# danbider/gp-quadrature

Measured on AMD Instinct MI355X. Metric: GP-fits/sec (fit + posterior mean at the N training points), N=1e6 d=2 SE kernel, higher is better.
Workload: dtype f64; 1 GPU; 2D squared-exponential l=0.2 var=2 sigma2=0.2, eps=1e-4, global N=1e6 synthetic (BASELINE configs[1] at the metric's N=1e6), points sharded over the GPUs; n_per_gpu=1000000, global_n=1000000, d=2, mtot=23, M=529, mean_cg_iters=68, parallelism=points sharded over 1 GPU(s), CG replicated

## Files before the change

### gp-quadrature_amd/csrc/cg_herm.hip

```cpp
#include <cstdlib>
#include <type_traits>

#include "cg_persistent_dev.hpp"
#include "spectral_weights.hpp"

namespace efgp {

namespace pcg {

namespace h64 {
constexpr int kThreadsH = 256, kWavesH = kThreadsH / 64;
constexpr int LDR = 72;
constexpr int LT = 40;
constexpr int LQ = 82;
constexpr int G_ELEMS = 16 * LDR, T_ELEMS = 32 * LT, Q_ELEMS = kWavesH * 8 * LQ;
constexpr int kLdsElems = G_ELEMS + T_ELEMS + Q_ELEMS;

__device__ __forceinline__ void dft8_in4_tail(double2 e0, double2 e1, double2 e2, double2 e3, double2 o0, double2 o1r, double2 o2r,
                                              double2 o3r, double2 (&v)[8]) {
    const double hh = 0.70710678118654752440;
    const double2 o1 = make_double2(hh * (o1r.x + o1r.y), hh * (o1r.y - o1r.x));
    const double2 o2 = mul_mi(o2r);
    const double2 o3 = make_double2(hh * (o3r.y - o3r.x), -hh * (o3r.x + o3r.y));
    v[0] = cadd(e0, o0);
// ... 320 lines not shown
    double2* const qw = Qb + (wave * 8 + ql) * LQ + 9 * jc;
    const double2* const qr = Qb + (wave * 8 + ql) * LQ + jc;

    double2 twr[7], twc[7];
#pragma unroll
    for (int t = 1; t < 8; ++t) {
        twr[t - 1] = a.g.tw[0][j * t];
        twc[t - 1] = a.g.tw[0][jc * t];
    }
    double sa[8], sb[8];
#pragma unroll
    for (int t = 0; t < 8; ++t) {
        const int f0 = jc + 8 * t;
        const double2 va = a.vhat[f0 * F + q], vb = a.vhat[f0 * F + q + 32];
        const double2 wa = a.g.tw[0][((n - 1) * (f0 + q)) & 63], wb = a.g.tw[0][((n - 1) * (f0 + q + 32)) & 63];
        sa[t] = 0.5 * (va.x * wa.x + va.y * wa.y);
        sb[t] = -0.5 * (vb.x * wb.x + vb.y * wb.y);
    }
    const bool z6_ok = jc > 0;

    hrow::RowLanes<8> L;
    L.setup<false>(a, row_role, k0, j);
    const double (&wsr)[KS] = L.wsr;

#ifdef EFGP_CG_STAMPS
    long long stamp_prev = (long long)__builtin_readcyclecounter();
#endif
    int stop = 0;
    double rcp_rz = 0.0;
    auto apply_A = [&](const double2 (&u)[KS], double2 (&Au)[KS]) __attribute__((always_inline)) {
        double2 v[8];
        EFGP_STAMP(7);
        if (row_role) {
            dft8_in4(make_double2(wsr[0] * u[0].x, wsr[0] * u[0].y), make_double2(wsr[1] * u[1].x, wsr[1] * u[1].y),
                     make_double2(wsr[2] * u[2].x, wsr[2] * u[2].y), make_double2(wsr[3] * u[3].x, wsr[3] * u[3].y), v);
            exchange_stage2(v, xw, xr, twr);
            s64::store8_all<8>(Gb + k0 * LDR + j, v);
        }
        __syncthreads();
        stop = s_stop;
        rcp_rz = s_rcp;
        if (stop) return;
        EFGP_STAMP(0);
        {
            const double2* g0 = Gb + q;
            const double2 a0 = g0[jc * LDR], b0 = g0[jc * LDR + 32];
            const double2 a1 = g0[(jc + 8) * LDR], b1 = g0[(jc + 8) * LDR + 32];
            const double2 a6 = g0[((16 - jc) & 15) * LDR], b6 = g0[((16 - jc) & 15) * LDR + 32];
            const double2 a7 = g0[(8 - jc) * LDR], b7 = g0[(8 - jc) * LDR + 32];
            const double2 z0 = jc == 0 ? make_double2(a0.x, b0.x) : make_double2(a0.x - b0.y, a0.y + b0.x);
            const double2 z1 = make_double2(a1.x - b1.y, a1.y + b1.x);
            double2 z6 = make_double2(a6.x + b6.y, b6.x - a6.y);
            const double2 z7 = make_double2(a7.x + b7.y, b7.x - a7.y);
            if (!z6_ok) z6 = make_double2(0.0, 0.0);
            dft8_in4(z0, z1, z6, z7, v);
            exchange_stage2(v, qw, qr, twc);
#pragma unroll
            for (int t = 0; t < 8; ++t) v[t] = make_double2(v[t].x * sa[t], v[t].y * sb[t]);
            dft_fwd<8>(v);
            exchange_stage2<true>(v, qw, qr, twc);
            double2* t0 = Tb + jc * LT + q;
            t0[0] = v[0];
            t0[8 * LT] = v[1];
            t0[16 * LT] = v[6];
            t0[24 * LT] = v[7];
        }
        __syncthreads();
        EFGP_STAMP(1);
        if (row_role) {
            const double2* tp = Tb + (k0 & 15) * LT + j;
            const double2* tm = Tb + ((k0 & 15) == 0 ? 0 : 32 - (k0 & 15)) * LT + j;
#pragma unroll
            for (int u4 = 0; u4 < 4; ++u4) {
                const double2 P = tp[8 * u4], Mv = tm[8 * u4];
                v[u4] = make_double2(P.x + Mv.x, P.y - Mv.y);
                v[u4 + 4] = make_double2(-P.y - Mv.y, P.x - Mv.x);
            }
            dft_fwd<8>(v);
            exchange_stage2<true>(v, xw, xr, twr);
            const double2 y[KS] = {s64::conjd(v[0]), s64::conjd(v[1]), s64::conjd(v[6]), s64::conjd(v[7])};
#pragma unroll
            for (int s = 0; s < KS; ++s) {
                const double2 gg = make_double2(wsr[s] * y[s].x, wsr[s] * y[s].y);
                if (VARIANT == 0) Au[s] = make_double2(gg.x + a.sigmasq * u[s].x, gg.y + a.sigmasq * u[s].y);
                else Au[s] = make_double2(gg.x / a.sigmasq + u[s].x, gg.y / a.sigmasq + u[s].y);
            }
        } else {
#pragma unroll
            for (int s = 0; s < KS; ++s) Au[s] = make_double2(0.0, 0.0);
        }
        EFGP_STAMP(2);
    };

    if (tid == 0) {
        s_stop = 0;
        s_rcp = 0.0;
    }
    double2 Ap[KS];
    if (a.zero_x0) {
#pragma unroll
        for (int s = 0; s < KS; ++s) Ap[s] = make_double2(0.0, 0.0);
    } else {
        apply_A(L.xv, Ap);
    }
    double rz, bb, asym;
    L.start(a, Ap, rz, bb, asym);
    block_sum_pair_h(rz, bb, red);
    asym = block_sum_h(asym, red);
    const double ws_bad = block_sum_h(L.ws_bad, red + kWavesH);
    if (hrow::refused(asym, bb, ws_bad)) {
        L.refuse(a);
        return;
    }
    const hrow::NormTest norm(bb);
    if (wave == 3 && lane == 0) s_rcp = 1.0 / (rz + 1e-16);
    int it = 0;
    for (; it < a.max_iter;) {
        apply_A(L.pv, Ap);
        if (stop) break;
        const double pAp = block_sum_h(L.dot_p(Ap), red) + 1e-16;
        EFGP_STAMP(3);
        const double alpha = rz / pAp;
        double rr, rzn;
        double2 zv[KS];
        L.step(alpha, Ap, zv, rr, rzn);
        EFGP_STAMP(4);
        block_sum_pair_h(rr, rzn, red);
        EFGP_STAMP(5);
        ++it;
        if (wave == 3) norm.publish(a, rr, rzn, it, lane, &s_rcp, &s_stop);
        L.new_direction(zv, rzn, rz, rcp_rz);
    }
    L.write_out(a, it);
}

namespace h48 {
constexpr int kThreadsH = 256, kWavesH = kThreadsH / 64;
constexpr int HF = 24, NR = 12;
constexpr int LDR = 56;
constexpr int LT = 28;
constexpr int LQ = 82;
constexpr int G_ELEMS = NR * LDR, T_ELEMS = 2 * NR * LT, Q_ELEMS = HF * LQ;
static_assert(NR * LX <= Q_ELEMS, "the row lines' scratch aliases the column lines' scratch");
constexpr int kLdsElems = G_ELEMS + T_ELEMS + Q_ELEMS;
constexpr int ND = 4 * F;
constexpr int NC = 25;
constexpr int kReread = 8;
constexpr int LDV = 49;
constexpr int kLdsElemsDense = F * LDV + (kThreadsH / 8) * LX;
static_assert(2 * G_ELEMS + NR * LX <= kLdsElemsDense, "the iteration's G, Yh and row scratch alias the prologue's grid");
constexpr int kThreadsP = 512, kRowWavesP = 2, kPairWavesP = 3;
constexpr int NDP = kThreadsP - 64 * kRowWavesP;
static_assert(NDP == 8 * F && 64 * kPairWavesP == 4 * F, "no wave mixes two-row and one-row groups");
constexpr int kLdsElemsPairs = F * LDV + (kThreadsP / 8) * LX;

__device__ __forceinline__ void exchange_8to6(const double2 (&v)[8], double2 (&u)[6], bool writer, double2* __restrict__ wr,
                                              const double2* __restrict__ rd, const double2 (&tw)[5]) {
    wave_sync();
    if (writer) s64::store8_all<1>(wr, v);
    wave_sync();
#pragma unroll
    for (int t = 0; t < 6; ++t) u[t] = rd[9 * t];
#pragma unroll
    for (int t = 1; t < 6; ++t) u[t] = cmulp(u[t], tw[t - 1]);
    dft6(u);
}
__device__ __forceinline__ double exchange_8to6_norm(const double2 (&v)[8], double2 (&u)[6], bool writer, double2* __restrict__ wr,
                                                     const double2* __restrict__ rd, const double2 (&tw)[5], const double2 (&x)[4],
                                                     double scale) {
    wave_sync();
    if (writer) s64::store8_all<1>(wr, v);
    wave_sync();
#pragma unroll
    for (int t = 0; t < 6; ++t) u[t] = rd[9 * t];
    __builtin_amdgcn_sched_barrier(0);
    const double x01 = fma(x[0].x, x[0].x, x[0].y * x[0].y) + fma(x[1].x, x[1].x, x[1].y * x[1].y);
    const double x23 = fma(x[2].x, x[2].x, x[2].y * x[2].y) + fma(x[3].x, x[3].x, x[3].y * x[3].y);
    const double xx = scale * (x01 + x23);
    __builtin_amdgcn_sched_barrier(0);
#pragma unroll
    for (int t = 1; t < 6; ++t) u[t] = cmulp(u[t], tw[t - 1]);
    dft6(u);
    return xx;
}
__device__ __forceinline__ void exchange_6to8(double2 (&u)[6], double2 (&v)[8], double2* __restrict__ wr, const double2* __restrict__ rd,
                                              const double2 (&tw)[5]) {
#pragma unroll
    for (int t = 1; t < 6; ++t) u[t] = cmulp(u[t], tw[t - 1]);
    wave_sync();
#pragma unroll
    for (int t = 0; t < 6; ++t) wr[t] = u[t];
    wave_sync();
    s64::load8_all<9>(rd, v);
    h64::dft8_out4(v);
}

__device__ __forceinline__ double half_wave_sum(double v) {
    EFGP_DPP_ADD(v, 0x111, 0xF);
    EFGP_DPP_ADD(v, 0x112, 0xF);
    EFGP_DPP_ADD(v, 0x114, 0xF);
    EFGP_DPP_ADD(v, 0x118, 0xF);
    EFGP_DPP_ADD(v, 0x142, 0xA);
    const int lo = __builtin_amdgcn_readlane(__double2loint(v), 31);
    const int hi = __builtin_amdgcn_readlane(__double2hiint(v), 31);
    return __hiloint2double(hi, lo);
}

template <bool LOW_ROUNDED>
__device__ __forceinline__ void dft8_in4_ws(const double (&w)[4], const double2 (&u)[4], double2 (&v)[8]) {
    constexpr int r0 = LOW_ROUNDED ? 0 : 2, r1 = LOW_ROUNDED ? 1 : 3, f0 = LOW_ROUNDED ? 2 : 0, f1 = LOW_ROUNDED ? 3 : 1;
    double2 e0, e1, e2, e3, o0, o1r, o2r, o3r;
    const double2 ra = make_double2(__dmul_rn(w[r0], u[r0].x), __dmul_rn(w[r0], u[r0].y));
    const double2 rb = make_double2(__dmul_rn(w[r1], u[r1].x), __dmul_rn(w[r1], u[r1].y));
    const double wa = w[f0], wb = w[f1];
    const double2 ua = u[f0], ub = u[f1];
    if constexpr (LOW_ROUNDED) {
        e0 = make_double2(fma(wa, ua.x, ra.x), fma(wa, ua.y, ra.y));
        e1 = make_double2(fma(-wa, ua.y, ra.x), fma(wa, ua.x, ra.y));
        e2 = make_double2(fma(-wa, ua.x, ra.x), fma(-wa, ua.y, ra.y));
        e3 = make_double2(fma(wa, ua.y, ra.x), fma(-wa, ua.x, ra.y));
        o0 = make_double2(fma(wb, ub.x, rb.x), fma(wb, ub.y, rb.y));
        o1r = make_double2(fma(-wb, ub.y, rb.x), fma(wb, ub.x, rb.y));
        o2r = make_double2(fma(-wb, ub.x, rb.x), fma(-wb, ub.y, rb.y));
        o3r = make_double2(fma(wb, ub.y, rb.x), fma(-wb, ub.x, rb.y));
    } else {
        e0 = make_double2(fma(wa, ua.x, ra.x), fma(wa, ua.y, ra.y));
        e1 = make_double2(fma(wa, ua.x, -ra.y), fma(wa, ua.y, ra.x));
        e2 = make_double2(fma(wa, ua.x, -ra.x), fma(wa, ua.y, -ra.y));
        e3 = make_double2(fma(wa, ua.x, ra.y), fma(wa, ua.y, -ra.x));
        o0 = make_double2(fma(wb, ub.x, rb.x), fma(wb, ub.y, rb.y));
        o1r = make_double2(fma(wb, ub.x, -rb.y), fma(wb, ub.y, rb.x));
        o2r = make_double2(fma(wb, ub.x, -rb.x), fma(wb, ub.y, -rb.y));
        o3r = make_double2(fma(wb, ub.x, rb.y), fma(wb, ub.y, -rb.x));
    }
    h64::dft8_in4_tail(e0, e1, e2, e3, o0, o1r, o2r, o3r, v);
}

__device__ __forceinline__ void wave_sum_pair(double& u, double& v) {
    EFGP_DPP_ADD(u, 0x111, 0xF);
    EFGP_DPP_ADD(v, 0x111, 0xF);
    EFGP_DPP_ADD(u, 0x112, 0xF);
    EFGP_DPP_ADD(v, 0x112, 0xF);
    EFGP_DPP_ADD(u, 0x114, 0xF);
    EFGP_DPP_ADD(v, 0x114, 0xF);
    EFGP_DPP_ADD(u, 0x118, 0xF);
    EFGP_DPP_ADD(v, 0x118, 0xF);
    EFGP_DPP_ADD(u, 0x142, 0xA);
    EFGP_DPP_ADD(v, 0x142, 0xA);
    EFGP_DPP_ADD(u, 0x143, 0xC);
    EFGP_DPP_ADD(v, 0x143, 0xC);
    const int ulo = __builtin_amdgcn_readlane(__double2loint(u), 63), uhi = __builtin_amdgcn_readlane(__double2hiint(u), 63);
    const int vlo = __builtin_amdgcn_readlane(__double2loint(v), 63), vhi = __builtin_amdgcn_readlane(__double2hiint(v), 63);
    u = __hiloint2double(uhi, ulo);
    v = __hiloint2double(vhi, vlo);
}

__device__ __forceinline__ double exchange_6to8_quot(double2 (&u)[6], double2 (&v)[8], double2* __restrict__ wr,
                                                     const double2* __restrict__ rd, const double2 (&tw)[5], double part, double num) {
#pragma unroll
    for (int t = 1; t < 6; ++t) u[t] = cmulp(u[t], tw[t - 1]);
    wave_sync();
#pragma unroll
    for (int t = 0; t < 6; ++t) wr[t] = u[t];
    wave_sync();
    s64::load8_all<9>(rd, v);
    __builtin_amdgcn_sched_barrier(0);
    const double quot = num / (half_wave_sum(part) + 1e-16);
    __builtin_amdgcn_sched_barrier(0);
    h64::dft8_out4(v);
    return quot;
}

template <int NT>
__device__ __forceinline__ void dense48_coeffs(double2* lds2, const double2 (&tw)[5], const double2* __restrict__ twg, int n,
                                               double2 (&cf)[NC]) {
    constexpr int SLOTS = NT / 8, PASSES = (F + SLOTS - 1) / SLOTS;
    double2* const buf = lds2;
    double2* const scr = lds2 + F * LDV;
    const int tid = threadIdx.x, slot = tid >> 3, j = tid & 7;
    double2* const wr = scr + slot * LX + 9 * j;
    const double2* const rd = scr + slot * LX + j;
    double2 u6[6], x8[8];
#pragma unroll
    for (int ps = 0; ps < PASSES; ++ps) {
        const int line = slot + ps * SLOTS;
        const bool act = line < F;
#pragma unroll
        for (int t = 0; t < 6; ++t) u6[t] = act ? s64::conjd(buf[(j + 8 * t) * LDV + line]) : make_double2(0.0, 0.0);
        dft6(u6);
#pragma unroll
        for (int t = 1; t < 6; ++t) u6[t] = cmulp(u6[t], tw[t - 1]);
        wave_sync();
#pragma unroll
        for (int t = 0; t < 6; ++t) wr[t] = u6[t];
        wave_sync();
        s64::load8_all<9>(rd, x8);
        dft_fwd<8>(x8);
        if (act && j < 6) {
#pragma unroll
            for (int t = 0; t < 8; ++t) buf[(j + 6 * t) * LDV + line] = s64::conjd(x8[t]);
        }
    }
    __syncthreads();
    const int f1 = tid % F, a0 = 3 * (tid / F);
    const bool dense = tid < ND;
    const double2 wc = twg[((n - 1) * f1) % F];
#pragma unroll
    for (int i = 0; i < NC; ++i) {
        const int l = a0 - 11 + i, al = l < 0 ? -l : l;
        double2 c = make_double2(0.0, 0.0);
        if (dense && al <= n - 1) {
            const double2 r = buf[(al + n - 1) * LDV + f1];
            c = make_double2(fma(r.y, wc.y, r.x * wc.x), fma(-r.x, wc.y, r.y * wc.x));
            if (l < 0) c.y = -c.y;
            if (l == 0) c.y = 0.0;
        }
        cf[i] = c;
    }
}

template <int NT>
__device__ __forceinline__ void dense48_inverse_pass(double2* lds2, const double2 (&tw)[5]) {
    constexpr int SLOTS = NT / 8, PASSES = (F + SLOTS - 1) / SLOTS;
    double2* const buf = lds2;
    double2* const scr = lds2 + F * LDV;
    const int tid = threadIdx.x, slot = tid >> 3, j = tid & 7;
    double2* const wr = scr + slot * LX + 9 * j;
    const double2* const rd = scr + slot * LX + j;
    double2 u6[6], x8[8];
#pragma unroll
    for (int ps = 0; ps < PASSES; ++ps) {
        const int line = slot + ps * SLOTS;
        const bool act = line < F;
#pragma unroll
        for (int t = 0; t < 6; ++t) u6[t] = act ? s64::conjd(buf[(j + 8 * t) * LDV + line]) : make_double2(0.0, 0.0);
        dft6(u6);
#pragma unroll
        for (int t = 1; t < 6; ++t) u6[t] = cmulp(u6[t], tw[t - 1]);
        wave_sync();
#pragma unroll
        for (int t = 0; t < 6; ++t) wr[t] = u6[t];
        wave_sync();
        s64::load8_all<9>(rd, x8);
        dft_fwd<8>(x8);
        if (act && j < 6) {
#pragma unroll
            for (int t = 0; t < 8; ++t) buf[(j + 6 * t) * LDV + line] = s64::conjd(x8[t]);
        }
    }
}
__device__ __forceinline__ double2 lag_coeff(const double2* buf, double2 wc, int n, int f1, int l) {
    const int al = l < 0 ? -l : l;
    double2 c = make_double2(0.0, 0.0);
    if (al <= n - 1) {
        const double2 r = buf[(al + n - 1) * LDV + f1];
        c = make_double2(fma(r.y, wc.y, r.x * wc.x), fma(-r.x, wc.y, r.y * wc.x));
        if (l < 0) c.y = -c.y;
        if (l == 0) c.y = 0.0;
    }
    return c;
}

constexpr int NM = NR - 1;
struct PairCoeffs {
    double2 c0;
    double2 S[NM], Q[NM];
};
__device__ __forceinline__ void pair_coeffs(const double2* buf, double2 wc, int n, int f1, int k0, PairCoeffs& pc) {
    pc.c0 = lag_coeff(buf, wc, n, f1, k0);
#pragma unroll
    for (int m = 1; m < NR; ++m) {
        const double2 cm = lag_coeff(buf, wc, n, f1, k0 - m), cp = lag_coeff(buf, wc, n, f1, k0 + m);
        pc.S[m - 1] = cadd(cm, cp);
        pc.Q[m - 1] = csub(cm, cp);
    }
}
__device__ __forceinline__ double2 pair_product(const PairCoeffs& pc, const double2 (&gm)[NR]) {
    double2 acc = make_double2(pc.c0.x * gm[0].x, pc.c0.y * gm[0].x);
#pragma unroll
    for (int m = 1; m < NR; ++m) {
        acc.x = fma(pc.S[m - 1].x, gm[m].x, acc.x);
        acc.y = fma(pc.S[m - 1].y, gm[m].x, acc.y);
        acc.x = fma(-pc.Q[m - 1].y, gm[m].y, acc.x);
        acc.y = fma(pc.Q[m - 1].x, gm[m].y, acc.y);
    }
    return acc;
}
}

template <int VARIANT, bool FUSED = false, bool DENSE = true, bool FREQ_DOT = false>
__global__ __launch_bounds__(h48::kThreadsH) void cg_herm48_kernel(Args a) {
    using namespace h48;
    using h64::block_sum_h;
    using h64::block_sum_pair_h;
    using h64::dft8_in4;
    using h64::div_rcp;
    constexpr int KS = 4;
    static_assert(h64::kWavesH == kWavesH, "the block reductions are shared with the 64 x 64 kernel");
    static_assert(DENSE || !FREQ_DOT, "the row-frequency <p,Ap> reads what the per-frequency Toeplitz products hold");
    extern __shared__ double2 lds2[];
    __shared__ double red[4 * kWavesH];
    __shared__ double s_rcp;
    __shared__ int s_stop;
    __shared__ double s_part[FREQ_DOT ? ND + 8 * NR : 1];
    double2* const Gb = lds2;
    double2* const Tb = lds2 + G_ELEMS;
    double2* const Qb = Tb + (DENSE ? G_ELEMS : T_ELEMS);
    const int n = a.g.n[0], h = (n - 1) / 2, M = a.g.M;
    const int row = blockIdx.x;
    const int64_t base = (int64_t)row * M;
    const int tid = threadIdx.x, lane = tid & 63, wave = tid >> 6;
    const int k0 = tid >> 3, j = tid & 7;
    const bool row_role = tid < 8 * NR, vec_role = row_role && j < 6;
    const int jc = lane >> 3, ql = lane & 7, q = wave * 8 + ql;
    const bool col_role = wave < 3, col6 = jc < 6;
    const int k0s = row_role ? k0 : 0;
    double2* const xw = Qb + k0s * LX + 9 * j;
    const double2* const xr = Qb + k0s * LX + j;
    const int qs = col_role ? q : 0;
    double2* const qw = Qb + qs * LQ + 9 * jc;
    const double2* const qr = Qb + qs * LQ + jc;
    const bool dense_role = tid < ND;
    const int f1d = tid % F, kd = 3 * (tid / F);
// ... 172 lines not shown
        if (row_role) {
            double uAu = 0.0;
            if constexpr (DENSE) {
                double pt[9];
                if constexpr (FREQ_DOT) {
                    const double* sp = s_part + (lane & 31);
#pragma unroll
                    for (int t = 0; t < 9; ++t) pt[t] = sp[32 * t];
                }
                const double2* tp = Tb + k0 * LDR + j;
#pragma unroll
                for (int t = 0; t < 6; ++t) u6[t] = tp[8 * t];
                if constexpr (FREQ_DOT) {
                    __builtin_amdgcn_sched_barrier(0);
                    double tsum = ((pt[0] + pt[1]) + (pt[2] + pt[3])) + (pt[4] + pt[5]);
                    if (VARIANT == 1) tsum /= a.sigmasq;
                    uAu = tsum + ((pt[6] + pt[7]) + pt[8]);
                }
            } else {
                const double2* tp = Tb + k0 * LT + j;
                const double2* tm = Tb + (k0 == 0 ? 0 : 2 * NR - k0) * LT + j;
#pragma unroll
                for (int u3 = 0; u3 < 3; ++u3) {
                    const double2 P = tp[8 * u3], Mv = tm[8 * u3];
                    u6[u3] = make_double2(P.x + Mv.x, P.y - Mv.y);
                    u6[u3 + 3] = make_double2(-P.y - Mv.y, P.x - Mv.x);
                }
            }
            dft6(u6);
            if constexpr (FREQ_DOT) alpha_fd = exchange_6to8_quot(u6, v, xw, xr, twr, uAu, rz);
            else exchange_6to8(u6, v, xw, xr, twr);
            const double2 y[KS] = {s64::conjd(v[0]), s64::conjd(v[1]), s64::conjd(v[6]), s64::conjd(v[7])};
#pragma unroll
            for (int s = 0; s < KS; ++s) {
                const double2 gg = make_double2(wsr[s] * y[s].x, wsr[s] * y[s].y);
                double2 val;
                if (VARIANT == 0) val = make_double2(gg.x + a.sigmasq * u[s].x, gg.y + a.sigmasq * u[s].y);
                else val = make_double2(gg.x / a.sigmasq + u[s].x, gg.y / a.sigmasq + u[s].y);
                Au[s] = ok[s] ? val : make_double2(0.0, 0.0);
            }
        } else {
            if constexpr (FREQ_DOT) alpha_fd = 0.0;
#pragma unroll
            for (int s = 0; s < KS; ++s) Au[s] = make_double2(0.0, 0.0);
        }
        EFGP_STAMP(2);
    };

    if (tid == 0) {
        s_stop = 0;
        s_rcp = 0.0;
    }
    double2 Ap[KS];
    if (a.zero_x0) {
#pragma unroll
        for (int s = 0; s < KS; ++s) Ap[s] = make_double2(0.0, 0.0);
    } else {
        apply_A(xv, Ap);
    }
    double bb = 0.0, asym = 0.0;
#pragma unroll
    for (int s = 0; s < KS; ++s) {
        if (ok[s]) {
            double2 bv = a.b[base + idx[s]];
            double2 bm = a.b[base + (M - 1 - idx[s])];
            if (a.b_times_ws) {
                bv = make_double2(wsr[s] * bv.x, wsr[s] * bv.y);
                bm = make_double2(wsr[s] * bm.x, wsr[s] * bm.y);
            }
            asym += (bv.x - bm.x) * (bv.x - bm.x) + (bv.y + bm.y) * (bv.y + bm.y);
            rv[s] = csub(bv, Ap[s]);
            pv[s] = precond ? make_double2(div_rcp(rv[s].x, dg[s], rdg[s]), div_rcp(rv[s].y, dg[s], rdg[s])) : rv[s];
            rz += rv[s].x * pv[s].x + rv[s].y * pv[s].y;
            bb += bv.x * bv.x + bv.y * bv.y;
        }
    }
    rz *= wgt;
    bb *= wgt;
    block_sum_pair_h(rz, bb, red);
    asym = block_sum_h(asym, red);
    ws_bad = block_sum_h(ws_bad, red + kWavesH);
    if (!(asym <= 1e-16 * bb) || ws_bad != 0.0) {
#pragma unroll
        for (int s = 0; s < KS; ++s) {
            if (ok[s]) {
                a.x[base + idx[s]] = make_double2(__builtin_nan(""), __builtin_nan(""));
                a.x[base + (M - 1 - idx[s])] = make_double2(__builtin_nan(""), __builtin_nan(""));
            }
        }
        if (tid == 0) a.iters[row] = -2;
        return;
    }
    const double bn = sqrt(bb);
    const double den = bn > 0.0 ? bn : 1.0;
    const double den_eps = den + 1e-16, rcp_den = 1.0 / den_eps;
    if (wave == 3 && lane == 0) s_rcp = 1.0 / (rz + 1e-16);
    int it = 0;
    for (; it < a.max_iter;) {
        apply_A(pv, Ap);
        if (stop) break;
        double alpha;
        if constexpr (FREQ_DOT) {
            alpha = alpha_fd;
        } else {
            double pAp = 0.0;
#pragma unroll
            for (int s = 0; s < KS; ++s) pAp += pv[s].x * Ap[s].x + pv[s].y * Ap[s].y;
            pAp = block_sum_h(pAp * wgt, red) + 1e-16;
            EFGP_STAMP(3);
            alpha = rz / pAp;
        }
        double rr = 0.0, rzn = 0.0;
        double2 zv[KS];
#pragma unroll
        for (int s = 0; s < KS; ++s) {
            xv[s].x += alpha * pv[s].x;
            xv[s].y += alpha * pv[s].y;
            rv[s].x -= alpha * Ap[s].x;
            rv[s].y -= alpha * Ap[s].y;
            zv[s] = precond ? make_double2(div_rcp(rv[s].x, dg[s], rdg[s]), div_rcp(rv[s].y, dg[s], rdg[s])) : rv[s];
            rr += rv[s].x * rv[s].x + rv[s].y * rv[s].y;
            rzn += rv[s].x * zv[s].x + rv[s].y * zv[s].y;
        }
        rr *= wgt;
        rzn *= wgt;
        EFGP_STAMP(4);
        block_sum_pair_h(rr, rzn, red);
        EFGP_STAMP(5);
        ++it;
        if (wave == 3) {
            const double ratio = div_rcp(sqrt(rr), den_eps, rcp_den);
            const bool conv = a.early_stop && ((ratio < a.tol) || (a.batched && sqrt(rr) < 1e-12));
            if (lane == 0) {
                if (a.hist && row == 0 && it <= a.hist_cap) a.hist[it - 1] = ratio;
                s_stop = conv ? 1 : 0;
                s_rcp = 1.0 / (rzn + 1e-16);
            }
        }
        const double beta = div_rcp(rzn, rz + 1e-16, rcp_rz);
#pragma unroll
        for (int s = 0; s < KS; ++s) pv[s] = make_double2(zv[s].x + beta * pv[s].x, zv[s].y + beta * pv[s].y);
        rz = rzn;
    }
#pragma unroll
    for (int s = 0; s < KS; ++s) {
        if (ok[s]) {
            a.x[base + idx[s]] = xv[s];
            if (k0 > 0) a.x[base + (M - 1 - idx[s])] = s64::conjd(xv[s]);
        }
    }
    if (tid == 0) a.iters[row] = it;
}

template <int NOUT>
__device__ __forceinline__ void pairs_dense_role(const Args& a, double2* lds2, double* red, double* s_part, double* s_rcp, int* s_stop) {
    using namespace h48;
    const double2* const Gb = lds2;
    double2* const Tb = lds2 + G_ELEMS;
    const int n = a.g.n[0];
    const int tid = threadIdx.x, lane = tid & 63, d = tid - 64 * kRowWavesP;
    const int f1d = d % F, grp = d / F, kd = NOUT == 2 ? 2 * grp : grp + 4;
    const bool duty = tid >= kThreadsP - 64;
    PairCoeffs pc[NOUT];
    {
        const double2 wc = a.g.tw[0][((n - 1) * f1d) % F];
#pragma unroll
        for (int o = 0; o < NOUT; ++o) pair_coeffs(lds2, wc, n, f1d, kd + o, pc[o]);
    }
    __syncthreads();
#ifdef EFGP_CG_STAMPS
    long long stamp_prev = 0;
#endif
    const double2* const g0 = Gb + f1d;
    double2* const t0 = Tb + kd * LDR + f1d;
    auto products = [&]() __attribute__((always_inline)) -> bool {
        __syncthreads();
#ifdef EFGP_CG_STAMPS
        EFGP_STAMP_RESTART(64 * kRowWavesP);
        const int flag = *s_stop;
        if (flag) return false;
#else
        if (*s_stop) return false;
#endif
        double2 gm[NR], acc[NOUT], gk[NOUT];
#pragma unroll
        for (int m = 0; m < NR; ++m) gm[m] = g0[m * LDR];
#ifdef EFGP_CG_STAMPS
        asm volatile("" ::"v"(gm[0].x), "v"(gm[0].y), "v"(flag));
        EFGP_STAMP_BY(8, 64 * kRowWavesP);
#endif
#pragma unroll
        for (int o = 0; o < NOUT; ++o) acc[o] = pair_product(pc[o], gm);
#pragma unroll
        for (int o = 0; o < NOUT; ++o) gk[o] = g0[(kd + o) * LDR];
        t0[0] = make_double2(acc[0].x, kd == 0 ? 0.0 : -acc[0].y);
        if constexpr (NOUT == 2) t0[LDR] = make_double2(acc[1].x, -acc[1].y);
        EFGP_STAMP_BY(1, 64 * kRowWavesP);
        const double t0r = kd == 0 ? gk[0].x * acc[0].x : 2.0 * fma(gk[0].y, acc[0].y, gk[0].x * acc[0].x);
        if constexpr (NOUT == 2) s_part[d] = fma(2.0, fma(gk[1].y, acc[1].y, gk[1].x * acc[1].x), t0r);
        else s_part[d] = t0r;
        __syncthreads();
        EFGP_STAMP_BY(6, 64 * kRowWavesP);
        return true;
    };
    if (!a.zero_x0) products();
    __syncthreads();
    const double rz = red[0] + red[4], bb = red[1] + red[5], asym = red[2] + red[6], ws_bad = red[3] + red[7];
    if (hrow::refused(asym, bb, ws_bad)) return;
    const hrow::NormTest norm(bb);
    if (duty && lane == 0) *s_rcp = 1.0 / (rz + 1e-16);
    for (int it = 0; it < a.max_iter;) {
        if (!products()) break;
        __syncthreads();
        ++it;
        if (duty) norm.publish(a, red[0] + red[1], red[2] + red[3], it, lane, s_rcp, s_stop);
    }
}

template <int VARIANT, bool FUSED = false, bool CHAIN_V1 = false, bool ROW_V1 = CHAIN_V1, bool PRECOND = true>
__global__ __launch_bounds__(h48::kThreadsP) void cg_herm48_pairs_kernel(Args a) {
    static_assert(ROW_V1 || !CHAIN_V1, "the statements of round 9 come with round 10's loop");
    using namespace h48;
    using h64::dft8_in4;
    using hrow::KS;
    extern __shared__ double2 lds2[];
    __shared__ double red[4 * kRowWavesP];
    __shared__ double s_rcp;
    __shared__ int s_stop;
    __shared__ double s_part[NDP + 8 * NR];
    double2* const Gb = lds2;
    double2* const Tb = lds2 + G_ELEMS;
    double2* const Qb = Tb + G_ELEMS;
    const int tid = threadIdx.x, lane = tid & 63;
    const int wave = __builtin_amdgcn_readfirstlane(tid >> 6);
    const int k0 = tid >> 3, j = tid & 7;

    double2 twr[5];
#pragma unroll
    for (int t = 1; t < 6; ++t) twr[t - 1] = a.g.tw[0][j * t];
    if (tid == 0) {
        s_stop = 0;
        s_rcp = 0.0;
    }
    constexpr bool EARLY = !CHAIN_V1, DEFER_X = !CHAIN_V1;
    [[maybe_unused]] hrow::EarlyLoads<6> early;
    if constexpr (EARLY) early.template issue<FUSED>(a, tid < 8 * NR && j < 6, k0, j);
    if (FUSED) {
        vhat48_lines<kThreadsP, true>(a.vsrc, a.vL0, a.vL1, 1.0 / 2304.0, a.vhat_out, lds2);
    } else {
#pragma unroll
        for (int k = 0; k < (F * F + kThreadsP - 1) / kThreadsP; ++k) {
            const int t = tid + k * kThreadsP, i0 = t / F, i1 = t - i0 * F;
            if (t < F * F) lds2[i0 * LDV + i1] = a.vhat[t];
        }
    }
    __syncthreads();
    dense48_inverse_pass<kThreadsP>(lds2, twr);
    __syncthreads();
    if (wave >= kRowWavesP + kPairWavesP) {
        pairs_dense_role<1>(a, lds2, red, s_part, &s_rcp, &s_stop);
        return;
    }
    if (wave >= kRowWavesP) {
        pairs_dense_role<2>(a, lds2, red, s_part, &s_rcp, &s_stop);
        return;
    }

    const bool row_role = tid < 8 * NR, vec_role = row_role && j < 6;
    const int k0s = row_role ? k0 : 0;
    double2* const xw = Qb + k0s * LX + 9 * j;
    const double2* const xr = Qb + k0s * LX + j;
    hrow::RowLanes<6> L;
    if constexpr (EARLY) L.template setup<FUSED, true>(a, vec_role, k0, j, &early);
    else L.template setup<FUSED>(a, vec_role, k0, j);
    const double (&wsr)[KS] = L.wsr;
    const bool (&ok)[KS] = L.ok;
    const double wgt = L.wgt;
    __syncthreads();
    if constexpr (!ROW_V1) {
        if (row_role && j >= 6) xw[6] = xw[7] = make_double2(0.0, 0.0);
    }

#ifdef EFGP_CG_STAMPS
    long long stamp_prev = (long long)__builtin_readcyclecounter();
#endif
    int stop = 0;
    double rcp_rz = 0.0;
    double rz = 0.0;
    double alpha_fd = 0.0;
    [[maybe_unused]] bool owed = false;
    [[maybe_unused]] double2 p_prev[KS];
    auto apply_A = [&](const double2 (&u)[KS], double2 (&Au)[KS], const double2 (&prev)[KS], auto first) __attribute__((always_inline)) {
        double2 v[8], u6[6];
        EFGP_STAMP(7);
        if (row_role) {
            if constexpr (ROW_V1)
                dft8_in4(make_double2(wsr[0] * u[0].x, wsr[0] * u[0].y), make_double2(wsr[1] * u[1].x, wsr[1] * u[1].y),
                         make_double2(wsr[2] * u[2].x, wsr[2] * u[2].y), make_double2(wsr[3] * u[3].x, wsr[3] * u[3].y), v);
            else
                dft8_in4_ws<!decltype(first)::value>(wsr, u, v);
            const double uu = exchange_8to6_norm(v, u6, j < 6, xw, xr, twr, u, VARIANT == 0 ? wgt * a.sigmasq : wgt);
            double2* g0 = Gb + k0 * LDR + j;
#pragma unroll
            for (int t = 0; t < 6; ++t) g0[8 * t] = u6[t];
            s_part[NDP + tid] = uu;
        }
        __syncthreads();
        stop = s_stop;
        rcp_rz = s_rcp;
        if (stop) return;
        EFGP_STAMP(0);
        if constexpr (DEFER_X) {
            if (owed) L.update_x(alpha_fd, prev);
            owed = false;
            if constexpr (ROW_V1) {
#pragma unroll
                for (int s = 0; s < KS; ++s) {
                    asm volatile("v_mov_b64 %0, %1" : "=v"(p_prev[s].x) : "v"(u[s].x));
                    asm volatile("v_mov_b64 %0, %1" : "=v"(p_prev[s].y) : "v"(u[s].y));
                }
            }
        }
        __syncthreads();
        EFGP_STAMP_RESTART(0);
        if (row_role) {
            double pt[15];
            const double* sp = s_part + (lane & 31);
#pragma unroll
            for (int t = 0; t < 15; ++t) pt[t] = sp[32 * t];
            const double2* tp = Tb + k0 * LDR + j;
#pragma unroll
            for (int t = 0; t < 6; ++t) u6[t] = tp[8 * t];
            __builtin_amdgcn_sched_barrier(0);
            double tsum = (((pt[0] + pt[1]) + (pt[2] + pt[3])) + ((pt[4] + pt[5]) + (pt[6] + pt[7]))) + ((pt[8] + pt[9]) + (pt[10] + pt[11]));
            if (VARIANT == 1) tsum /= a.sigmasq;
            const double uAu = tsum + ((pt[12] + pt[13]) + pt[14]);
            dft6(u6);
            alpha_fd = exchange_6to8_quot(u6, v, xw, xr, twr, uAu, rz);
            const double2 y[KS] = {s64::conjd(v[0]), s64::conjd(v[1]), s64::conjd(v[6]), s64::conjd(v[7])};
#pragma unroll
            for (int s = 0; s < KS; ++s) {
                const double2 gg = make_double2(wsr[s] * y[s].x, wsr[s] * y[s].y);
                double2 val;
                if (VARIANT == 0) val = make_double2(gg.x + a.sigmasq * u[s].x, gg.y + a.sigmasq * u[s].y);
                else val = make_double2(gg.x / a.sigmasq + u[s].x, gg.y / a.sigmasq + u[s].y);
                if constexpr (!ROW_V1 && VARIANT == 0)
                    Au[s] = make_double2(fma(a.sigmasq, u[s].x, __dmul_rn(wsr[s], y[s].x)), fma(a.sigmasq, u[s].y, __dmul_rn(wsr[s], y[s].y)));
                else if constexpr (!ROW_V1) Au[s] = val;
                else Au[s] = ok[s] ? val : make_double2(0.0, 0.0);
            }
        } else {
            alpha_fd = 0.0;
#pragma unroll
            for (int s = 0; s < KS; ++s) Au[s] = make_double2(0.0, 0.0);
        }
        EFGP_STAMP(2);
    };

    double2 Ap[KS];
    if (a.zero_x0) {
#pragma unroll
        for (int s = 0; s < KS; ++s) Ap[s] = make_double2(0.0, 0.0);
    } else {
        apply_A(L.xv, Ap, p_prev, std::true_type{});
    }
    double bb, asym;
    if constexpr (EARLY) L.template start<true>(a, Ap, rz, bb, asym, &early);
    else L.start(a, Ap, rz, bb, asym);
    rz = wave_sum(rz);
    bb = wave_sum(bb);
    asym = wave_sum(asym);
    double ws_bad = wave_sum(L.ws_bad);
    if (lane == 0) {
        red[4 * wave] = rz;
        red[4 * wave + 1] = bb;
        red[4 * wave + 2] = asym;
        red[4 * wave + 3] = ws_bad;
    }
    __syncthreads();
    rz = red[0] + red[4];
    bb = red[1] + red[5];
    asym = red[2] + red[6];
    ws_bad = red[3] + red[7];
    if (hrow::refused(asym, bb, ws_bad)) {
        L.refuse(a);
        return;
    }
    int it = 0;
    if constexpr (!ROW_V1) {
        double2 p_alt[KS];
#pragma unroll
        for (int s = 0; s < KS; ++s) p_alt[s] = make_double2(0.0, 0.0);
        auto half = [&](const double2 (&pc)[KS], double2 (&pn)[KS]) __attribute__((always_inline)) -> bool {
            apply_A(pc, Ap, pn, std::false_type{});
            if (stop) return false;
            double rr, rzn;
            double2 zv[KS];
            L.template step_<PRECOND, false>(alpha_fd, Ap, zv, rr, rzn);
            owed = true;
            EFGP_STAMP(4);
            wave_sum_pair(rr, rzn);
            if (lane == 0) {
                red[wave] = rr;
                red[2 + wave] = rzn;
            }
            __syncthreads();
            rzn = red[2] + red[3];
            EFGP_STAMP(5);
            ++it;
            L.new_direction_to(zv, rzn, rz, rcp_rz, pc, pn);
            return true;
        };
        bool owed_alt = false;
        for (;;) {
            owed_alt = true;
            if (it >= a.max_iter || !half(L.pv, p_alt)) break;
            owed_alt = false;
            if (it >= a.max_iter || !half(p_alt, L.pv)) break;
        }
        if (owed) L.update_x(alpha_fd, owed_alt ? p_alt : L.pv);
        L.write_out(a, it);
        return;
    }
    for (; it < a.max_iter;) {
        apply_A(L.pv, Ap, p_prev, std::false_type{});
        if (stop) break;
        double rr, rzn;
        double2 zv[KS];
        if constexpr (DEFER_X) {
            L.template step<false>(alpha_fd, Ap, zv, rr, rzn);
            owed = true;
        } else {
            L.step(alpha_fd, Ap, zv, rr, rzn);
        }
        EFGP_STAMP(4);
        rr = wave_sum(rr);
        rzn = wave_sum(rzn);
        if (lane == 0) {
            red[wave] = rr;
            red[2 + wave] = rzn;
        }
        __syncthreads();
        rzn = red[2] + red[3];
        EFGP_STAMP(5);
        ++it;
        L.new_direction(zv, rzn, rz, rcp_rz);
    }
    if constexpr (DEFER_X) {
        if (owed) L.update_x(alpha_fd, p_prev);
    }
    L.write_out(a, it);
}

static void operands48(const Herm48Operands& h48, const MeanFusedOperands* fuse, Args& a) {
    a.vhat = fuse ? nullptr : h48.vhat;
    a.g.F[0] = a.g.F[1] = 48;
    a.g.tw[0] = a.g.tw[1] = h48.tw;
    if (!fuse) return;
    a.ws = nullptr;
    a.wk_kind = fuse->kind;
    a.wk_mtot = fuse->mtot;
    a.wk_nu = fuse->nu;
    a.wk_ell = fuse->ell;
    a.wk_c0 = fuse->c0;
    a.wk_h = fuse->h;
    a.ws_out = fuse->ws_out;
    a.vsrc = fuse->v;
    a.vL0 = fuse->L0;
    a.vL1 = fuse->L1;
    a.vhat_out = fuse->vhat48_out;
}

PickLaunch herm_launch(const PersistentChoice& c, int variant, const Herm48Operands* h48, const MeanFusedOperands* fuse, Args& a) {
    if (c.pick == PersistentPick::fused48 || c.pick == PersistentPick::herm48) operands48(*h48, fuse, a);
    constexpr size_t lds48d = (size_t)h48::kLdsElemsDense * sizeof(double2);
    static_assert(h48::kLdsElemsDense >= h48::kLdsElems, "the fused prologue's LDS covers the iteration's");
    const bool freq_dot = std::getenv("EFGP_CG48_MODE_DOT") == nullptr;
    const bool pairs = c.dense48 && freq_dot && std::getenv("EFGP_CG48_LAG_COEFFS") == nullptr;
    constexpr size_t lds48p = (size_t)h48::kLdsElemsPairs * sizeof(double2);
    const bool chain_v1 = std::getenv("EFGP_CG48_CHAIN_V1") != nullptr;
    const int arm = chain_v1 ? 3 : (std::getenv("EFGP_CG48_ROW_V1") != nullptr ? 2 : (hrow::has_precond(a) ? 0 : 1));
    static const char* const fused8[4] = {"fused mean solve (48x48, eight waves)", "fused mean solve (48x48, eight waves, no diagonal)",
                                          "fused mean solve (48x48, eight waves, row role of round 10)",
                                          "fused mean solve (48x48, eight waves, round 9)"};
    static const char* const herm8[4] = {"persistent CG (48x48, Hermitian, eight waves)", "persistent CG (48x48, Hermitian, eight waves, no diagonal)",
                                         "persistent CG (48x48, Hermitian, eight waves, row role of round 10)",
                                         "persistent CG (48x48, Hermitian, eight waves, round 9)"};
    switch (c.pick) {
        case PersistentPick::fused48: {
            if (pairs) {
                void (*const eight[4])(Args) = {cg_herm48_pairs_kernel<0, true>, cg_herm48_pairs_kernel<0, true, false, false, false>,
                                                cg_herm48_pairs_kernel<0, true, false, true>, cg_herm48_pairs_kernel<0, true, true>};
                return {eight[arm], h48::kThreadsP, lds48p, fused8[arm]};
            }
            void (*const dense[2])(Args) = {cg_herm48_kernel<0, true, true, false>, cg_herm48_kernel<0, true, true, true>};
            return {c.dense48 ? dense[freq_dot] : cg_herm48_kernel<0, true, false>, h48::kThreadsH, lds48d, "fused mean solve (48x48)"};
        }
        case PersistentPick::herm48: {
            if (pairs) {
                void (*const eight[4][2])(Args) = {{cg_herm48_pairs_kernel<0>, cg_herm48_pairs_kernel<1>},
                                                   {cg_herm48_pairs_kernel<0, false, false, false, false>, cg_herm48_pairs_kernel<1, false, false, false, false>},
                                                   {cg_herm48_pairs_kernel<0, false, false, true>, cg_herm48_pairs_kernel<1, false, false, true>},
                                                   {cg_herm48_pairs_kernel<0, false, true>, cg_herm48_pairs_kernel<1, false, true>}};
                return {eight[arm][variant != 0], h48::kThreadsP, lds48p, herm8[arm]};
            }
            void (*const dense[2][2])(Args) = {{cg_herm48_kernel<0, false, true, false>, cg_herm48_kernel<1, false, true, false>},
                                               {cg_herm48_kernel<0, false, true, true>, cg_herm48_kernel<1, false, true, true>}};
            void (*const fft2d[2])(Args) = {cg_herm48_kernel<0, false, false>, cg_herm48_kernel<1, false, false>};
            return {(c.dense48 ? dense[freq_dot] : fft2d)[variant != 0], h48::kThreadsH,
                    c.dense48 ? lds48d : (size_t)h48::kLdsElems * sizeof(double2), "persistent CG (48x48, Hermitian)"};
        }
        default:
            break;
    }
    return {variant == 0 ? cg_herm64_kernel<0> : cg_herm64_kernel<1>, h64::kThreadsH, (size_t)h64::kLdsElems * sizeof(double2),
            "persistent CG (64x64, Hermitian)"};
}

}

}
```

Baseline: 5183 GP fits/s of the global N=1e6 problem (whole job; the points are sharded over the GPUs).

## Compute CG step length on a spare dense wave instead of the row waves

Moves the uAu reduction and the alpha = rz/uAu division from the row-role waves onto a dedicated one-row dense wave, which publishes alpha through shared memory. The row waves now run the inverse 6-to-8 exchange without the reduction on their path. The norm share is computed after the stop check rather than inside the exchange, and the accumulator zeroing is hoisted out of the loop. This costs an extra block barrier per iteration, and the alpha wave must also track rz. A fused-FMA DFT8 tail is used on this path too, and an env var restores the old arrangement.

```diff
diff --git a/gp-quadrature_amd/csrc/cg_herm.hip b/gp-quadrature_amd/csrc/cg_herm.hip
--- a/gp-quadrature_amd/csrc/cg_herm.hip
+++ b/gp-quadrature_amd/csrc/cg_herm.hip
@@ -496,6 +496,8 @@
 constexpr int kThreadsP = 512, kRowWavesP = 2, kPairWavesP = 3;
 constexpr int NDP = kThreadsP - 64 * kRowWavesP;
 static_assert(NDP == 8 * F && 64 * kPairWavesP == 4 * F, "no wave mixes two-row and one-row groups");
+constexpr int kAlphaWaveP = 7;
+static_assert(kAlphaWaveP >= kRowWavesP + kPairWavesP && kAlphaWaveP < kThreadsP / 64, "a wave of the one-row dense role");
 constexpr int kLdsElemsPairs = F * LDV + (kThreadsP / 8) * LX;
 
 __device__ __forceinline__ void exchange_8to6(const double2 (&v)[8], double2 (&u)[6], bool writer, double2* __restrict__ wr,
@@ -508,6 +510,11 @@
 #pragma unroll
     for (int t = 1; t < 6; ++t) u[t] = cmulp(u[t], tw[t - 1]);
     dft6(u);
+}
+__device__ __forceinline__ double norm_share(const double2 (&x)[4], double scale) {
+    const double x01 = fma(x[0].x, x[0].x, x[0].y * x[0].y) + fma(x[1].x, x[1].x, x[1].y * x[1].y);
+    const double x23 = fma(x[2].x, x[2].x, x[2].y * x[2].y) + fma(x[3].x, x[3].x, x[3].y * x[3].y);
+    return scale * (x01 + x23);
 }
 __device__ __forceinline__ double exchange_8to6_norm(const double2 (&v)[8], double2 (&u)[6], bool writer, double2* __restrict__ wr,
                                                      const double2* __restrict__ rd, const double2 (&tw)[5], const double2 (&x)[4],
@@ -549,8 +556,24 @@
     const int hi = __builtin_amdgcn_readlane(__double2hiint(v), 31);
     return __hiloint2double(hi, lo);
 }
-
-template <bool LOW_ROUNDED>
+__device__ __forceinline__ double quot_half_wave(double part, double num) { return num / (half_wave_sum(part) + 1e-16); }
+
+__device__ __forceinline__ void dft8_in4_tail_fused(double2 e0, double2 e1, double2 e2, double2 e3, double2 o0, double2 o1r, double2 o2r,
+                                                    double2 o3r, double2 (&v)[8]) {
+    const double hh = 0.70710678118654752440;
+    const double s1 = o1r.x + o1r.y, d1 = o1r.y - o1r.x, s3 = o3r.x + o3r.y, d3 = o3r.y - o3r.x;
+    const double2 o2 = mul_mi(o2r);
+    v[0] = cadd(e0, o0);
+    v[4] = csub(e0, o0);
+    v[1] = make_double2(fma(hh, s1, e1.x), fma(hh, d1, e1.y));
+    v[5] = make_double2(fma(-hh, s1, e1.x), fma(-hh, d1, e1.y));
+    v[2] = cadd(e2, o2);
+    v[6] = csub(e2, o2);
+    v[3] = make_double2(fma(hh, d3, e3.x), fma(-hh, s3, e3.y));
+    v[7] = make_double2(fma(-hh, d3, e3.x), fma(hh, s3, e3.y));
+}
+
+template <bool LOW_ROUNDED, bool FUSED_TAIL = false>
 __device__ __forceinline__ void dft8_in4_ws(const double (&w)[4], const double2 (&u)[4], double2 (&v)[8]) {
     constexpr int r0 = LOW_ROUNDED ? 0 : 2, r1 = LOW_ROUNDED ? 1 : 3, f0 = LOW_ROUNDED ? 2 : 0, f1 = LOW_ROUNDED ? 3 : 1;
     double2 e0, e1, e2, e3, o0, o1r, o2r, o3r;
@@ -577,7 +600,8 @@
         o2r = make_double2(fma(wb, ub.x, -rb.x), fma(wb, ub.y, -rb.y));
         o3r = make_double2(fma(wb, ub.x, rb.y), fma(wb, ub.y, -rb.x));
     }
-    h64::dft8_in4_tail(e0, e1, e2, e3, o0, o1r, o2r, o3r, v);
+    if constexpr (FUSED_TAIL) dft8_in4_tail_fused(e0, e1, e2, e3, o0, o1r, o2r, o3r, v);
+    else h64::dft8_in4_tail(e0, e1, e2, e3, o0, o1r, o2r, o3r, v);
 }
 
 __device__ __forceinline__ void wave_sum_pair(double& u, double& v) {
@@ -609,10 +633,22 @@
     wave_sync();
     s64::load8_all<9>(rd, v);
     __builtin_amdgcn_sched_barrier(0);
-    const double quot = num / (half_wave_sum(part) + 1e-16);
+    const double quot = quot_half_wave(part, num);
     __builtin_amdgcn_sched_barrier(0);
     h64::dft8_out4(v);
     return quot;
+}
+
+__device__ __forceinline__ void uAu_summands(const double* s_part, int lane, double (&pt)[15]) {
+    const double* sp = s_part + (lane & 31);
+#pragma unroll
+    for (int t = 0; t < 15; ++t) pt[t] = sp[32 * t];
+}
+template <int VARIANT>
+__device__ __forceinline__ double uAu_of_lane(const double (&pt)[15], double sigmasq) {
+    double tsum = (((pt[0] + pt[1]) + (pt[2] + pt[3])) + ((pt[4] + pt[5]) + (pt[6] + pt[7]))) + ((pt[8] + pt[9]) + (pt[10] + pt[11]));
+    if (VARIANT == 1) tsum /= sigmasq;
+    return tsum + ((pt[12] + pt[13]) + pt[14]);
 }
 
 template <int NT>
@@ -1091,8 +1127,9 @@
     if (tid == 0) a.iters[row] = it;
 }
 
-template <int NOUT>
-__device__ __forceinline__ void pairs_dense_role(const Args& a, double2* lds2, double* red, double* s_part, double* s_rcp, int* s_stop) {
+template <int NOUT, int VARIANT, bool ALPHA_WAVE>
+__device__ __forceinline__ void pairs_dense_role(const Args& a, double2* lds2, double* red, double* s_part, double* s_rcp, int* s_stop,
+                                                 double* s_alpha) {
     using namespace h48;
     const double2* const Gb = lds2;
     double2* const Tb = lds2 + G_ELEMS;
@@ -1100,6 +1137,7 @@
     const int tid = threadIdx.x, lane = tid & 63, d = tid - 64 * kRowWavesP;
     const int f1d = d % F, grp = d / F, kd = NOUT == 2 ? 2 * grp : grp + 4;
     const bool duty = tid >= kThreadsP - 64;
+    [[maybe_unused]] const bool sums = NOUT == 1 && tid >> 6 == kAlphaWaveP;
     PairCoeffs pc[NOUT];
     {
         const double2 wc = a.g.tw[0][((n - 1) * f1d) % F];
@@ -1112,7 +1150,7 @@
 #endif
     const double2* const g0 = Gb + f1d;
     double2* const t0 = Tb + kd * LDR + f1d;
-    auto products = [&]() __attribute__((always_inline)) -> bool {
+    auto products = [&]([[maybe_unused]] double rz) __attribute__((always_inline)) -> bool {
         __syncthreads();
 #ifdef EFGP_CG_STAMPS
         EFGP_STAMP_RESTART(64 * kRowWavesP);
@@ -1140,25 +1178,39 @@
         else s_part[d] = t0r;
         __syncthreads();
         EFGP_STAMP_BY(6, 64 * kRowWavesP);
+        if constexpr (ALPHA_WAVE) {
+            if (sums) {
+                double pt[15];
+                uAu_summands(s_part, lane, pt);
+                const double alpha = quot_half_wave(uAu_of_lane<VARIANT>(pt, a.sigmasq), rz);
+                if (lane == 0) *s_alpha = alpha;
+            }
+            __syncthreads();
+        }
         return true;
     };
-    if (!a.zero_x0) products();
+    if (!a.zero_x0) products(0.0);
     __syncthreads();
-    const double rz = red[0] + red[4], bb = red[1] + red[5], asym = red[2] + red[6], ws_bad = red[3] + red[7];
+    double rz = red[0] + red[4];
+    const double bb = red[1] + red[5], asym = red[2] + red[6], ws_bad = red[3] + red[7];
     if (hrow::refused(asym, bb, ws_bad)) return;
     const hrow::NormTest norm(bb);
     if (duty && lane == 0) *s_rcp = 1.0 / (rz + 1e-16);
     for (int it = 0; it < a.max_iter;) {
-        if (!products()) break;
+        if (!products(rz)) break;
         __syncthreads();
         ++it;
         if (duty) norm.publish(a, red[0] + red[1], red[2] + red[3], it, lane, s_rcp, s_stop);
-    }
-}
-
-template <int VARIANT, bool FUSED = false, bool CHAIN_V1 = false, bool ROW_V1 = CHAIN_V1, bool PRECOND = true>
+        if constexpr (ALPHA_WAVE) {
+            if (sums) rz = red[2] + red[3];
+        }
+    }
+}
+
+template <int VARIANT, bool FUSED = false, bool CHAIN_V1 = false, bool ROW_V1 = CHAIN_V1, bool PRECOND = true, bool ALPHA_WAVE = !ROW_V1>
 __global__ __launch_bounds__(h48::kThreadsP) void cg_herm48_pairs_kernel(Args a) {
     static_assert(ROW_V1 || !CHAIN_V1, "the statements of round 9 come with round 10's loop");
+    static_assert(!ALPHA_WAVE || !ROW_V1, "the step length on a dense wave comes with round 11's row role");
     using namespace h48;
     using h64::dft8_in4;
     using hrow::KS;
@@ -1167,6 +1219,7 @@
     __shared__ double s_rcp;
     __shared__ int s_stop;
     __shared__ double s_part[NDP + 8 * NR];
+    __shared__ double s_alpha;
     double2* const Gb = lds2;
     double2* const Tb = lds2 + G_ELEMS;
     double2* const Qb = Tb + G_ELEMS;
@@ -1182,6 +1235,8 @@
         s_rcp = 0.0;
     }
     constexpr bool EARLY = !CHAIN_V1, DEFER_X = !CHAIN_V1;
+    constexpr bool UU_GAP = ALPHA_WAVE;
+    constexpr bool ZEROS_ONCE = ALPHA_WAVE;
     [[maybe_unused]] hrow::EarlyLoads<6> early;
     if constexpr (EARLY) early.template issue<FUSED>(a, tid < 8 * NR && j < 6, k0, j);
     if (FUSED) {
@@ -1197,11 +1252,11 @@
     dense48_inverse_pass<kThreadsP>(lds2, twr);
     __syncthreads();
     if (wave >= kRowWavesP + kPairWavesP) {
-        pairs_dense_role<1>(a, lds2, red, s_part, &s_rcp, &s_stop);
+        pairs_dense_role<1, VARIANT, ALPHA_WAVE>(a, lds2, red, s_part, &s_rcp, &s_stop, &s_alpha);
         return;
     }
     if (wave >= kRowWavesP) {
-        pairs_dense_role<2>(a, lds2, red, s_part, &s_rcp, &s_stop);
+        pairs_dense_role<2, VARIANT, ALPHA_WAVE>(a, lds2, red, s_part, &s_rcp, &s_stop, &s_alpha);
         return;
     }
 
@@ -1237,12 +1292,14 @@
                 dft8_in4(make_double2(wsr[0] * u[0].x, wsr[0] * u[0].y), make_double2(wsr[1] * u[1].x, wsr[1] * u[1].y),
                          make_double2(wsr[2] * u[2].x, wsr[2] * u[2].y), make_double2(wsr[3] * u[3].x, wsr[3] * u[3].y), v);
             else
-                dft8_in4_ws<!decltype(first)::value>(wsr, u, v);
-            const double uu = exchange_8to6_norm(v, u6, j < 6, xw, xr, twr, u, VARIANT == 0 ? wgt * a.sigmasq : wgt);
+                dft8_in4_ws<!decltype(first)::value, ALPHA_WAVE>(wsr, u, v);
+            double uu = 0.0;
+            if constexpr (UU_GAP) exchange_8to6(v, u6, j < 6, xw, xr, twr);
+            else uu = exchange_8to6_norm(v, u6, j < 6, xw, xr, twr, u, VARIANT == 0 ? wgt * a.sigmasq : wgt);
             double2* g0 = Gb + k0 * LDR + j;
 #pragma unroll
             for (int t = 0; t < 6; ++t) g0[8 * t] = u6[t];
-            s_part[NDP + tid] = uu;
+            if constexpr (!UU_GAP) s_part[NDP + tid] = uu;
         }
         __syncthreads();
         stop = s_stop;
@@ -1260,22 +1317,12 @@
                 }
             }
         }
+        if constexpr (UU_GAP) {
+            if (row_role) s_part[NDP + tid] = norm_share(u, VARIANT == 0 ? wgt * a.sigmasq : wgt);
+        }
         __syncthreads();
         EFGP_STAMP_RESTART(0);
-        if (row_role) {
-            double pt[15];
-            const double* sp = s_part + (lane & 31);
-#pragma unroll
-            for (int t = 0; t < 15; ++t) pt[t] = sp[32 * t];
-            const double2* tp = Tb + k0 * LDR + j;
-#pragma unroll
-            for (int t = 0; t < 6; ++t) u6[t] = tp[8 * t];
-            __builtin_amdgcn_sched_barrier(0);
-            double tsum = (((pt[0] + pt[1]) + (pt[2] + pt[3])) + ((pt[4] + pt[5]) + (pt[6] + pt[7]))) + ((pt[8] + pt[9]) + (pt[10] + pt[11]));
-            if (VARIANT == 1) tsum /= a.sigmasq;
-            const double uAu = tsum + ((pt[12] + pt[13]) + pt[14]);
-            dft6(u6);
-            alpha_fd = exchange_6to8_quot(u6, v, xw, xr, twr, uAu, rz);
+        auto form_Au = [&]() __attribute__((always_inline)) {
             const double2 y[KS] = {s64::conjd(v[0]), s64::conjd(v[1]), s64::conjd(v[6]), s64::conjd(v[7])};
 #pragma unroll
             for (int s = 0; s < KS; ++s) {
@@ -1288,7 +1335,33 @@
                 else if constexpr (!ROW_V1) Au[s] = val;
                 else Au[s] = ok[s] ? val : make_double2(0.0, 0.0);
             }
-        } else {
+        };
+        if constexpr (ALPHA_WAVE) {
+            if (row_role) {
+                const double2* tp = Tb + k0 * LDR + j;
+#pragma unroll
+                for (int t = 0; t < 6; ++t) u6[t] = tp[8 * t];
+                dft6(u6);
+                exchange_6to8(u6, v, xw, xr, twr);
+            }
+            __syncthreads();
+        }
+        if (row_role) {
+            if constexpr (ALPHA_WAVE) {
+                alpha_fd = s_alpha;
+            } else {
+                double pt[15];
+                uAu_summands(s_part, lane, pt);
+                const double2* tp = Tb + k0 * LDR + j;
+#pragma unroll
+                for (int t = 0; t < 6; ++t) u6[t] = tp[8 * t];
+                __builtin_amdgcn_sched_barrier(0);
+                const double uAu = uAu_of_lane<VARIANT>(pt, a.sigmasq);
+                dft6(u6);
+                alpha_fd = exchange_6to8_quot(u6, v, xw, xr, twr, uAu, rz);
+            }
+            form_Au();
+        } else if constexpr (!ZEROS_ONCE) {
             alpha_fd = 0.0;
 #pragma unroll
             for (int s = 0; s < KS; ++s) Au[s] = make_double2(0.0, 0.0);
@@ -1297,12 +1370,11 @@
     };
 
     double2 Ap[KS];
-    if (a.zero_x0) {
+    if (a.zero_x0 || ZEROS_ONCE) {
 #pragma unroll
         for (int s = 0; s < KS; ++s) Ap[s] = make_double2(0.0, 0.0);
-    } else {
-        apply_A(L.xv, Ap, p_prev, std::true_type{});
-    }
+    }
+    if (!a.zero_x0) apply_A(L.xv, Ap, p_prev, std::true_type{});
     double bb, asym;
     if constexpr (EARLY) L.template start<true>(a, Ap, rz, bb, asym, &early);
     else L.start(a, Ap, rz, bb, asym);
@@ -1418,18 +1490,30 @@
     const bool pairs = c.dense48 && freq_dot && std::getenv("EFGP_CG48_LAG_COEFFS") == nullptr;
     constexpr size_t lds48p = (size_t)h48::kLdsElemsPairs * sizeof(double2);
     const bool chain_v1 = std::getenv("EFGP_CG48_CHAIN_V1") != nullptr;
-    const int arm = chain_v1 ? 3 : (std::getenv("EFGP_CG48_ROW_V1") != nullptr ? 2 : (hrow::has_precond(a) ? 0 : 1));
-    static const char* const fused8[4] = {"fused mean solve (48x48, eight waves)", "fused mean solve (48x48, eight waves, no diagonal)",
+    const bool alpha_rows = std::getenv("EFGP_CG48_ALPHA_ROWS") != nullptr;
+    const int arm =
+        chain_v1 ? 3 : (std::getenv("EFGP_CG48_ROW_V1") != nullptr ? 2 : (hrow::has_precond(a) ? 0 : 1) + (alpha_rows ? 4 : 0));
+    static const char* const fused8[6] = {"fused mean solve (48x48, eight waves)",
+                                          "fused mean solve (48x48, eight waves, no diagonal)",
                                           "fused mean solve (48x48, eight waves, row role of round 10)",
-                                          "fused mean solve (48x48, eight waves, round 9)"};
-    static const char* const herm8[4] = {"persistent CG (48x48, Hermitian, eight waves)", "persistent CG (48x48, Hermitian, eight waves, no diagonal)",
+                                          "fused mean solve (48x48, eight waves, round 9)",
+                                          "fused mean solve (48x48, eight waves, step length on the row waves)",
+                                          "fused mean solve (48x48, eight waves, no diagonal, step length on the row waves)"};
+    static const char* const herm8[6] = {"persistent CG (48x48, Hermitian, eight waves)",
+                                         "persistent CG (48x48, Hermitian, eight waves, no diagonal)",
                                          "persistent CG (48x48, Hermitian, eight waves, row role of round 10)",
-                                         "persistent CG (48x48, Hermitian, eight waves, round 9)"};
+                                         "persistent CG (48x48, Hermitian, eight waves, round 9)",
+                                         "persistent CG (48x48, Hermitian, eight waves, step length on the row waves)",
+                                         "persistent CG (48x48, Hermitian, eight waves, no diagonal, step length on the row waves)"};
     switch (c.pick) {
         case PersistentPick::fused48: {
             if (pairs) {
-                void (*const eight[4])(Args) = {cg_herm48_pairs_kernel<0, true>, cg_herm48_pairs_kernel<0, true, false, false, false>,
-                                                cg_herm48_pairs_kernel<0, true, false, true>, cg_herm48_pairs_kernel<0, true, true>};
+                void (*const eight[6])(Args) = {cg_herm48_pairs_kernel<0, true>,
+                                                cg_herm48_pairs_kernel<0, true, false, false, false>,
+                                                cg_herm48_pairs_kernel<0, true, false, true>,
+                                                cg_herm48_pairs_kernel<0, true, true>,
+                                                cg_herm48_pairs_kernel<0, true, false, false, true, false>,
+                                                cg_herm48_pairs_kernel<0, true, false, false, false, false>};
                 return {eight[arm], h48::kThreadsP, lds48p, fused8[arm]};
             }
             void (*const dense[2])(Args) = {cg_herm48_kernel<0, true, true, false>, cg_herm48_kernel<0, true, true, true>};
@@ -1437,10 +1521,13 @@
         }
         case PersistentPick::herm48: {
             if (pairs) {
-                void (*const eight[4][2])(Args) = {{cg_herm48_pairs_kernel<0>, cg_herm48_pairs_kernel<1>},
-                                                   {cg_herm48_pairs_kernel<0, false, false, false, false>, cg_herm48_pairs_kernel<1, false, false, false, false>},
-                                                   {cg_herm48_pairs_kernel<0, false, false, true>, cg_herm48_pairs_kernel<1, false, false, true>},
-                                                   {cg_herm48_pairs_kernel<0, false, true>, cg_herm48_pairs_kernel<1, false, true>}};
+                void (*const eight[6][2])(Args) = {
+                    {cg_herm48_pairs_kernel<0>, cg_herm48_pairs_kernel<1>},
+                    {cg_herm48_pairs_kernel<0, false, false, false, false>, cg_herm48_pairs_kernel<1, false, false, false, false>},
+                    {cg_herm48_pairs_kernel<0, false, false, true>, cg_herm48_pairs_kernel<1, false, false, true>},
+                    {cg_herm48_pairs_kernel<0, false, true>, cg_herm48_pairs_kernel<1, false, true>},
+                    {cg_herm48_pairs_kernel<0, false, false, false, true, false>, cg_herm48_pairs_kernel<1, false, false, false, true, false>},
+                    {cg_herm48_pairs_kernel<0, false, false, false, false, false>, cg_herm48_pairs_kernel<1, false, false, false, false, false>}};
                 return {eight[arm][variant != 0], h48::kThreadsP, lds48p, herm8[arm]};
             }
             void (*const dense[2][2])(Args) = {{cg_herm48_kernel<0, false, true, false>, cg_herm48_kernel<1, false, true, false>},
```

Result: faster. 5363 GP fits/s of the global N=1e6 problem (whole job; the points are sharded over the GPUs), median of 6 (+3.5%).
